# reasv/panoptikon

Measured on AMD Instinct MI355X. Metric: knn_queries_per_sec, higher is better.
Workload: dtype i8

## Files before the change

panoptikon_amd/csrc/pvs_api.hip:

```cpp
#include "pvs_index.hpp"

static thread_local std::string g_last_error;

pvs_status pvs_fail(pvs_status code, const char *fmt, ...) {
    char buf[512];
    va_list ap;
    va_start(ap, fmt);
    vsnprintf(buf, sizeof buf, fmt, ap);
    va_end(ap);
    g_last_error = buf;
    return code;
}
PVS_EXPORT const char *pvs_last_error(void) { return g_last_error.c_str(); }

namespace {
std::atomic<int64_t> g_dbg[PVS_DBG_COUNT];
const char *const g_dbg_names[PVS_DBG_COUNT] = {
    "sample_div",      "sample_j_div", "no_light_finalize", "force_light_finalize", "dense_per_query",     "no_direct_score",
    "no_page_rank",    "rrf_serial",   "rrf_full",          "rrf_trace",            "scan_no_wide128",     "scratch_idle_cap_mb",
    "scratch_bypass",  "rrf_digest",   "no_sparse",         "sparse_max",           "no_fused_agg",        "no_side_finalize",
    "rrf_host_rounds", "multi_host_pages", "prelude_stream", "dense_nq4", "marker_events", "no_direct_topk", "direct_max_mb", "direct_queries",
    "direct_unit", "direct_static_pct", "direct_max_nq", "dense_full_sort", "dense_page_first", "no_flag_poll", "poll_late_pages",
    "no_exact_wide", "no_agg8", "no_dense2", "comm_timeout_s", "comm_fail_local",
    "no_float_certify", "float_certify_queries", "float_certify_rows", "float_certify_trace", "float_certify_no_fold",
// ... 285 lines not shown
    }
    c.spans.clear();
    c.span_pool.clear();
    hipFree(c.d_qin);
    hipFree(c.d_qmat);
    hipFree(c.d_qpad);
    hipFree(c.d_direct);
    hipFree(c.d_qstage);
    hipFree(c.d_mask);
    hipFree(c.d_aux_masked);
    hipFree(c.d_qexact);
    hipFree(c.d_qinfo);
    hipFree(c.d_thr);
    hipFree(c.d_gmin);
    hipFree(c.d_cand_cnt);
    hipFree(c.d_seg);
    hipFree(c.d_seg_cnt);
    hipFree(c.d_cand);
    hipFree(c.d_flat_cnt);
    hipFree(c.d_fin_ub);
    hipFree(c.d_fin_surv);
    hipFree(c.d_fin_sort);
    c.d_fin_ub = c.d_fin_surv = nullptr;
    c.d_fin_sort = nullptr;
    hipFree(c.d_need_dense);
    if (c.h_need_dense) hipHostFree(c.h_need_dense);
    hipFree(c.d_out_ids);
    hipFree(c.d_out_dist);
    hipFree(c.d_out_count);
    pvs_dense_release(c.dense);
    pvs_group_work_release(c.gwork);
    if (c.done) hipEventDestroy(c.done);
    if (c.scanned) hipEventDestroy(c.scanned);
    if (c.preluded) hipEventDestroy(c.preluded);
    hipFree(c.d_loc_rec);
    hipFree(c.d_all_rec);
    if (c.h_all_flags) hipHostFree(c.h_all_flags);
    if (c.own_stream) hipStreamDestroy(c.own_stream);
    if (c.h_io) hipHostFree(c.h_io);
    if (c.h_cert) hipHostFree(c.h_cert);
    c = SearchCtx();
}

pvs_status ctx_pinned_io(SearchCtx &c, size_t bytes) {
    if (bytes <= c.h_io_cap) return PVS_OK;
    if (c.h_io) hipHostFree(c.h_io);
    c.h_io = nullptr;
    c.h_io_cap = 0;
    const size_t cap = pvs_round_up(std::max<size_t>(bytes, 1 << 16), 1 << 16);
    HIP_TRY(hipHostMalloc((void **)&c.h_io, cap, hipHostMallocDefault));
    c.h_io_cap = cap;
    return PVS_OK;
}

pvs_status ctx_fin_buffers(SearchCtx &c) {
    if (c.d_fin_ub && c.d_fin_surv && c.d_fin_sort) return PVS_OK;
    if (!c.d_fin_ub) HIP_TRY(pvs_malloc_retry((void **)&c.d_fin_ub, 4 * (size_t)PVS_SCAN_MAX_BATCH * PVS_CAND_CAP));
    if (!c.d_fin_surv) HIP_TRY(pvs_malloc_retry((void **)&c.d_fin_surv, 4 * (size_t)PVS_SCAN_MAX_BATCH * PVS_SURV_CAP));
    if (!c.d_fin_sort) HIP_TRY(pvs_malloc_retry((void **)&c.d_fin_sort, 8 * (size_t)PVS_SCAN_MAX_BATCH * PVS_SURV_CAP));
    return PVS_OK;
}

pvs_status ctx_prepare(pvs_index *ix, SearchCtx &c, uint32_t batch, uint32_t k, bool host_outputs) {
    if (ix->multi_stream) {
        if (!c.own_stream) HIP_TRY(hipStreamCreateWithFlags(&c.own_stream, hipStreamNonBlocking));
        c.stream = c.own_stream;
    } else {
        c.stream = ix->search_stream;
    }
    c.cur_mask = nullptr;
    if (!c.done) HIP_TRY(hipEventCreateWithFlags(&c.done, hipEventDisableTiming));
    if (!c.scanned) HIP_TRY(hipEventCreateWithFlags(&c.scanned, hipEventDisableTiming));
    if (!c.preluded) HIP_TRY(hipEventCreateWithFlags(&c.preluded, hipEventDisableTiming));
    c.side_finalize = false;
    if (!c.d_qmat) {
        HIP_TRY(pvs_malloc_retry((void **)&c.d_qin, (size_t)PVS_SCAN_MAX_BATCH * ix->dim * 4));
        HIP_TRY(pvs_malloc_retry((void **)&c.d_qmat, (size_t)PVS_SCAN_MAX_BATCH * ix->stride));
        HIP_TRY(pvs_malloc_retry((void **)&c.d_qpad, pvs_dense_exact_scratch_bytes(ix->stride, ix->esz)));
        HIP_TRY(pvs_malloc_retry((void **)&c.d_qexact, (size_t)PVS_SCAN_MAX_BATCH * ix->dim * 4));
        HIP_TRY(pvs_malloc_retry((void **)&c.d_qinfo, sizeof(QInfo) * PVS_SCAN_MAX_BATCH));
        HIP_TRY(pvs_malloc_retry((void **)&c.d_thr, 4 * PVS_SCAN_MAX_BATCH));
        HIP_TRY(pvs_malloc_retry((void **)&c.d_gmin, (size_t)4 * PVS_SCAN_MAX_BATCH * GMAX));
        HIP_TRY(pvs_malloc_retry((void **)&c.d_cand_cnt, 64));
        HIP_TRY(pvs_malloc_retry((void **)&c.d_seg, sizeof(uint2) * (size_t)PVS_SEG_PAIRS * PVS_SEG_CAP));
        HIP_TRY(pvs_malloc_retry((void **)&c.d_seg_cnt, 4 * (size_t)PVS_SEG_PAIRS * (PVS_SEG_CAP / PVS_WIDE_SEG_CAP)));
        HIP_TRY(pvs_malloc_retry((void **)&c.d_cand, sizeof(uint2) * (size_t)PVS_SCAN_MAX_BATCH * PVS_CAND_CAP));
        HIP_TRY(pvs_malloc_retry((void **)&c.d_flat_cnt, 4 * (size_t)PVS_SCAN_MAX_BATCH));
    }
    if (batch > c.flags_cap) {
        hipFree(c.d_need_dense);
        if (c.h_need_dense) hipHostFree(c.h_need_dense);
        c.d_need_dense = nullptr;
        c.h_need_dense = nullptr;
        uint32_t cap = (uint32_t)pvs_round_up(batch, 256);
        HIP_TRY(pvs_malloc_retry((void **)&c.d_need_dense, 8 * (size_t)cap));
        HIP_TRY(hipHostMalloc((void **)&c.h_need_dense, 8 * (size_t)cap, hipHostMallocDefault));
        c.flags_cap = cap;
    }
    if (host_outputs) {
        uint64_t need = (uint64_t)batch * k;
        if (need > c.out_cap || batch > c.out_batch_cap) {
            hipFree(c.d_out_ids);
            hipFree(c.d_out_dist);
            hipFree(c.d_out_count);
// ... 592 lines not shown
```

panoptikon_amd/csrc/pvs_index.hpp:

```cpp
#pragma once
#include <sched.h>

#include <algorithm>
#include <cmath>
#include <chrono>
#include <condition_variable>
#include <thread>

#include "pvs_kernels.hpp"

struct PendingChunk {
    uint32_t qoff, nb;
};

struct PageSplit {
    uint32_t at;
    int64_t *ids;
    float *dist;
    uint32_t *count, *h_flags, *h_seen;
};

struct TimedSpan {
    hipEvent_t a, b;
    int kind;
    uint64_t rows;
};

struct SearchCtx {
    std::vector<TimedSpan> spans;
    std::vector<TimedSpan> span_pool;
    hipStream_t stream = nullptr;
    hipStream_t own_stream = nullptr;
    hipEvent_t done = nullptr;
    hipEvent_t preluded = nullptr;
    hipEvent_t scanned = nullptr;
    bool side_finalize = false;
    bool busy = false;
    bool draining = false, finished = false;
    pvs_status fin_status = PVS_OK;
    std::string fin_err;
    uint8_t *d_qin = nullptr;
    uint8_t *d_qmat = nullptr;
    float *d_qpad = nullptr;
    void *d_direct = nullptr;
    const uint8_t *cur_mask = nullptr;
    uint8_t *d_mask = nullptr;
    float *d_aux_masked = nullptr;
    uint64_t mask_cap = 0;
    void *d_qstage = nullptr;
    size_t qstage_cap = 0;
    uint8_t *d_qexact = nullptr;
    QInfo *d_qinfo = nullptr;
    float *d_thr = nullptr;
    float *d_gmin = nullptr;
    uint32_t *d_cand_cnt = nullptr;
    uint2 *d_seg = nullptr;
    uint32_t *d_seg_cnt = nullptr;
    uint2 *d_cand = nullptr;
    uint32_t *d_flat_cnt = nullptr;
    uint32_t *d_fin_ub = nullptr, *d_fin_surv = nullptr;
    unsigned long long *d_fin_sort = nullptr;
    uint32_t *d_need_dense = nullptr;
    uint32_t *h_need_dense = nullptr;
    uint32_t flags_cap = 0;
    int64_t *d_out_ids = nullptr;
    float *d_out_dist = nullptr;
    uint32_t *d_out_count = nullptr;
    uint64_t out_cap = 0;
    uint32_t out_batch_cap = 0;
// ... 362 lines not shown
```

panoptikon_amd/csrc/pvs_kernels.hpp:

```cpp
#pragma once
#include <cstring>
#include "pvs_common.hpp"

hipError_t pvs_launch_norm2(int dtype, const uint8_t *rows, uint32_t stride, uint32_t dim, uint64_t row0, uint64_t n,
                            float *norm2, float *rnorm, hipStream_t s);
hipError_t pvs_launch_fill_f32(float *p, uint64_t n, float v, hipStream_t s);
hipError_t pvs_launch_scan_aux(const float *norm2, const float *rnorm, uint64_t row0, uint64_t n, float *scan_cos, float *scan_l2,
                               hipStream_t s);
hipError_t pvs_launch_rows_ingest(int mode, const void *src, uint32_t dim, uint32_t esz, uint64_t row0, uint64_t n, float scale,
                                  uint8_t *rows, uint32_t stride, hipStream_t s);
hipError_t pvs_launch_rows_gather(const uint8_t *rows, uint32_t stride, uint32_t row_bytes, uint64_t row0, uint64_t n, uint8_t *dst,
                                  hipStream_t s);
hipError_t pvs_launch_pick_rows(const void *src, uint32_t row_bytes, const uint32_t *idx, uint64_t m, void *dst, hipStream_t s);
hipError_t pvs_launch_rows_to_queries(int dtype, const uint8_t *rows, uint32_t stride, uint32_t dim, const uint32_t *idx, uint32_t m, void *out, hipStream_t s);
hipError_t pvs_launch_take_rows(const void *in, uint32_t elem_bytes, const uint32_t *global_row, uint64_t n_local, void *out, hipStream_t s);
hipError_t pvs_launch_quantize_flat(const float *src, uint64_t n, float scale, int8_t *dst, hipStream_t s);
hipError_t pvs_launch_absmax(const float *src, uint64_t n, float *d_out_bits, hipStream_t s);
hipError_t pvs_launch_synth(uint64_t seed, uint64_t row0, uint64_t n, uint32_t dim, float *out, hipStream_t s);
hipError_t pvs_launch_synth_clustered(uint64_t seed, uint64_t row0, uint64_t n, uint32_t dim, float *out, hipStream_t s);
hipError_t pvs_launch_iota_ids(int64_t *ids, uint64_t n, int64_t base, hipStream_t s);

hipError_t pvs_launch_prep_queries(int index_dtype, int qdtype, const void *queries, uint32_t batch,
                                   uint32_t batch_pad, uint32_t dim, uint32_t stride, float scale,
                                   int metric, uint8_t *qmat, void *qexact, QInfo *qinfo, uint32_t *need_dense, hipStream_t s);
// ... 97 lines not shown

hipError_t pvs_launch_void_thresholds(float *thr, const uint32_t *need_dense, uint32_t n, hipStream_t s);

hipError_t pvs_launch_kth(const float *vals, uint32_t per_query, uint32_t batch, uint32_t k, float *out,
                          hipStream_t s, const QInfo *qinfo = nullptr, int metric = 0);

struct FinalizeArgs {
    int dtype, metric;
    const uint8_t *rows;
    const float *norm2;
    const int64_t *ids;
    uint32_t stride, dim;
    uint64_t n_rows;
    const void *qexact;
    const QInfo *qinfo;
    const uint2 *seg;
    const uint32_t *seg_cnt;
    uint32_t n_segments, seg_queries;
    uint32_t seg_cap = PVS_SEG_CAP;
    uint2 *cand;
    uint32_t cand_cap;
    uint32_t batch, k;
    int64_t *out_ids;
    float *out_dist;
    uint32_t *out_count;
    uint32_t *need_dense;
    uint32_t *cand_seen = nullptr;
    const uint32_t *flat_cnt = nullptr;
    const float *thr = nullptr;
    const float *thr_all = nullptr;
    int null_ok = 0;
    uint32_t *h_flags = nullptr, *h_seen = nullptr;
    uint32_t split = UINT32_MAX;
    int64_t *out_ids2 = nullptr;
    float *out_dist2 = nullptr;
    uint32_t *out_count2 = nullptr, *h_flags2 = nullptr, *h_seen2 = nullptr;
    const uint32_t *trank = nullptr, *tinv = nullptr;
    uint32_t *w_ub = nullptr;
    uint32_t *w_surv = nullptr;
    unsigned long long *w_sort = nullptr;
    hipEvent_t ev_start = nullptr, ev_stop = nullptr;
};
hipError_t pvs_launch_finalize(const FinalizeArgs &a, hipStream_t s);

struct DenseWork {
    float *d_dist = nullptr;
    uint32_t *d_keys_in = nullptr, *d_keys_out = nullptr, *d_vals_in = nullptr, *d_vals_out = nullptr;
    void *d_temp = nullptr;
    size_t temp_bytes = 0;
    uint64_t cap_rows = 0, sort_rows = 0;
    uint32_t *d_sample = nullptr, *d_sample_out = nullptr, *d_ctl = nullptr, *h_ctl = nullptr;
    unsigned long long *d_comp = nullptr, *d_comp_out = nullptr;
    void *d_temp_page = nullptr;
    size_t temp_page_bytes = 0;
    uint32_t comp_cap = 0;
};
pvs_status pvs_dense_reserve(DenseWork &w, uint64_t n);
void pvs_dense_release(DenseWork &w);
struct DenseBounds {
    int have_gt = 0, have_lt = 0;
    double gt = 0.0, lt = 0.0;
};
pvs_status pvs_dense_topk(DenseWork &w, uint64_t n, uint32_t k, const int64_t *ids, int64_t *out_ids,
                          float *out_dist, uint32_t *out_count, hipStream_t s, const uint8_t *mask = nullptr,
                          DenseBounds bounds = DenseBounds(), const uint32_t *tinv = nullptr);
pvs_status pvs_build_tie_ranks(const int64_t *d_keys, uint64_t n, uint32_t *d_trank, uint32_t *d_tinv, hipStream_t s);
// ... 111 lines not shown
```

panoptikon_amd/csrc/pvs_kernels_scan.hip:

```cpp
#include <cstdlib>

#include <hip/hip_ext.h>
#include "pvs_kernels.hpp"
#include "pvs_rerank.hpp"
#include "pvs_scan_dispatch.hpp"

bool pvs_scan_supported(int dtype, uint32_t kslabs) {
    if (dtype == PVS_I8) return (kslabs >= 1 && kslabs <= 6) || kslabs == 8 || kslabs == 12;
    if (dtype == PVS_F16)
        return kslabs == 1 || kslabs == 2 || kslabs == 3 || kslabs == 4 || kslabs == 6 || kslabs == 8 || kslabs == 9 || kslabs == 10 || kslabs == 12;
    if (dtype == PVS_F32)
        return kslabs == 1 || kslabs == 2 || kslabs == 3 || kslabs == 4 || kslabs == 6 || kslabs == 8 || kslabs == 12 || kslabs == 16 || kslabs == 18 ||
               kslabs == 20 || kslabs == 24;
    return false;
}
bool pvs_scan_is_wide(int dtype, uint32_t qgroups, uint32_t kslabs) {
    const bool no128 = pvs_dbg(PVS_DBG_SCAN_NO_WIDE128) != 0;
    if (dtype != PVS_I8 || (qgroups == 4 && no128)) return false;
    return pvs_scan_wide_serves(qgroups, kslabs, 1);
}
uint32_t pvs_scan_wg_rows(int dtype, uint32_t qgroups, uint32_t kslabs) {
    if (pvs_scan_is_wide(dtype, qgroups, kslabs)) return pvs_scan_wide_rows(kslabs);
    return qgroups >= 4 ? 32u : 32u * (4u / qgroups);
}
// ... 235 lines not shown
    }
}

hipError_t pvs_launch_kth(const float *vals, uint32_t per_query, uint32_t batch, uint32_t k, float *out, hipStream_t s, const QInfo *qinfo, int metric) {
    const uint32_t bp = (batch + 31) / 32 * 32;
    hipLaunchKernelGGL(k_kth, dim3(bp), dim3(256), 0, s, vals, per_query, batch, k, out, qinfo, metric);
    return hipGetLastError();
}

struct FinK {
    const uint8_t *rows;
    const float *norm2;
    const int64_t *ids;
    const void *qexact;
    const QInfo *qinfo;
    const uint2 *seg;
    const uint32_t *seg_cnt;
    uint2 *cand;
    int64_t *out_ids;
    float *out_dist;
    uint32_t *out_count, *need_dense, *cand_seen;
    uint64_t n_rows;
    uint32_t stride, dim, cand_cap, k, n_segments, seg_queries, seg_cap;
    int metric;
    uint32_t *w_ub, *w_surv;
    unsigned long long *w_sort;
    const uint32_t *flat_cnt;
    const float *thr;
    const float *thr_all;
    int null_ok;
    uint32_t *h_flags, *h_seen;
    const uint32_t *trank, *tinv;
    uint32_t split;
    int64_t *out_ids2;
    float *out_dist2;
    uint32_t *out_count2, *h_flags2, *h_seen2;
};

constexpr int FIN_QMAX = 8192;
constexpr int FIN_LDS = PVS_CAND_CAP * 4 + PVS_SURV_CAP * 4 + 64 + FIN_QMAX;

__device__ static inline float cand_err(const FinK &a, const QInfo &qi, float aa) {
    return a.metric == PVS_COSINE ? qi.eA : qi.eA + qi.eR * aa;
}
template <int DT>
__device__ static inline float cand_key(const FinK &a, const QInfo &qi, uint32_t payload, float aa) {
    if constexpr (DT == PVS_I8) {
        const float d = (float)(int)payload;
        return a.metric == PVS_COSINE ? -d * __frcp_rn(__fsqrt_rn(aa)) : aa + (qi.bb - 2.0f * d);
    } else {
        return __builtin_bit_cast(float, payload);
    }
}

constexpr uint32_t FIN_SMALL_SORT = 512;
template <int DT, bool LIGHT>
__global__ __launch_bounds__(256) void k_finalize(FinK a) {
    extern __shared__ __attribute__((aligned(16))) uint8_t smem[];
    __shared__ uint32_t hist[256];
    __shared__ uint32_t s_misc_light[LIGHT ? 16 : 1];
    __shared__ unsigned long long s_sort_light[LIGHT ? FIN_SMALL_SORT : 1];
    const uint32_t q = blockIdx.x;
    uint32_t *const s_ub = LIGHT ? a.w_ub + (size_t)q * a.cand_cap : (uint32_t *)smem;
    uint32_t *const s_surv = LIGHT ? a.w_surv + (size_t)q * PVS_SURV_CAP : (uint32_t *)(smem + PVS_CAND_CAP * 4);
    uint32_t *const s_misc = LIGHT ? s_misc_light : (uint32_t *)(smem + PVS_CAND_CAP * 4) + PVS_SURV_CAP;
    unsigned long long *s_sort = LIGHT ? s_sort_light : (unsigned long long *)smem;

    const int tid = threadIdx.x;
#ifdef PVS_FIN_PROF
    unsigned long long fp[8] = {0, 0, 0, 0, 0, 0, 0, 0};
#define FIN_STAMP(i) fp[i] = __builtin_amdgcn_s_memrealtime()
#else
#define FIN_STAMP(i) do { } while (0)
#endif
    FIN_STAMP(0);
    const bool second = q >= a.split;
    const uint32_t qo = second ? q - a.split : q;
    uint32_t *const out_count = second ? a.out_count2 : a.out_count;
    uint32_t *const h_flags = second ? a.h_flags2 : a.h_flags;
    uint32_t *const h_seen = second ? a.h_seen2 : a.h_seen;
    int64_t *oid = (second ? a.out_ids2 : a.out_ids) + (size_t)qo * a.k;
    float *od = (second ? a.out_dist2 : a.out_dist) + (size_t)qo * a.k;
    if (a.null_ok && !a.flat_cnt && pvs_query_all_null(a.metric, a.qinfo[q].bb)) {
        if (tid == 0) {
            a.need_dense[q] = 3;
            if (h_flags) h_flags[qo] = 3;
            out_count[qo] = 0;
            if (a.cand_seen) a.cand_seen[q] = 0;
            if (h_seen) h_seen[qo] = 0;
        }
        return;
    }
    uint2 *const flat = a.cand + (size_t)q * a.cand_cap;
    constexpr uint32_t FIN_STAGE = 4096;
    static_assert(FIN_STAGE * 8 * 2 <= PVS_CAND_CAP * 4 && FIN_STAGE * 2 <= PVS_SURV_CAP, "staging areas overlap");
// ... 270 lines not shown
            oid[i] = -1;
            od[i] = __builtin_nanf("");
        }
    }
    if (tid == 0) {
        out_count[qo] = nout;
        a.need_dense[q] = tail ? 3 : 0;
        if (h_flags) h_flags[qo] = tail ? 3 : 0;
    }
}

hipError_t pvs_launch_finalize(const FinalizeArgs &f, hipStream_t s) {
    FinK k;
    k.rows = f.rows;
    k.norm2 = f.norm2;
    k.ids = f.ids;
    k.qexact = f.qexact;
    k.qinfo = f.qinfo;
    k.seg = f.seg;
    k.seg_cnt = f.seg_cnt;
    k.n_segments = f.n_segments;
    k.w_ub = f.w_ub;
    k.w_surv = f.w_surv;
    k.w_sort = f.w_sort;
    k.seg_queries = f.seg_queries;
    k.seg_cap = f.seg_cap;
    k.flat_cnt = f.flat_cnt;
    k.thr = f.thr;
    k.thr_all = f.thr_all;
    k.null_ok = f.null_ok;
    k.h_flags = f.h_flags;
    k.h_seen = f.h_seen;
    k.split = f.split;
    k.out_ids2 = f.out_ids2;
    k.out_dist2 = f.out_dist2;
    k.out_count2 = f.out_count2;
    k.h_flags2 = f.h_flags2;
    k.h_seen2 = f.h_seen2;
    k.trank = f.trank;
    k.tinv = f.tinv;
    k.cand = f.cand;
    k.out_ids = f.out_ids;
    k.out_dist = f.out_dist;
    k.out_count = f.out_count;
    k.need_dense = f.need_dense;
    k.cand_seen = f.cand_seen;
    k.n_rows = f.n_rows;
    k.stride = f.stride;
    k.dim = f.dim;
    k.cand_cap = f.cand_cap;
    k.k = f.k;
    k.metric = f.metric;
    static std::atomic<bool> configured{false};
    if (!configured.load(std::memory_order_acquire)) {
        hipError_t e = hipFuncSetAttribute((const void *)k_finalize<PVS_I8, false>, hipFuncAttributeMaxDynamicSharedMemorySize, FIN_LDS);
        if (e == hipSuccess)
            e = hipFuncSetAttribute((const void *)k_finalize<PVS_F16, false>, hipFuncAttributeMaxDynamicSharedMemorySize, FIN_LDS);
        if (e == hipSuccess)
            e = hipFuncSetAttribute((const void *)k_finalize<PVS_F32, false>, hipFuncAttributeMaxDynamicSharedMemorySize, FIN_LDS);
        if (e != hipSuccess) return e;
        configured.store(true, std::memory_order_release);
    }
    if ((((uint64_t)f.dim * (f.dtype == PVS_I8 ? 1u : 4u)) + 63u & ~63ull) > (uint64_t)FIN_QMAX) return hipErrorInvalidValue;
    const bool light = f.w_ub && f.w_surv && f.w_sort;
    const size_t qlds = ((size_t)f.dim * 4 + 63) & ~(size_t)63;
#define PVS_FIN_LAUNCH(kernel, lds)                                                                                  \
    do {                                                                                                             \
        if (f.ev_start || f.ev_stop)                                                                                 \
            hipExtLaunchKernelGGL(kernel, dim3(f.batch), dim3(256), lds, s, f.ev_start, f.ev_stop, 0, k);            \
        else                                                                                                         \
            hipLaunchKernelGGL(kernel, dim3(f.batch), dim3(256), lds, s, k);                                         \
    } while (0)
    if (light && f.dtype == PVS_I8)
        PVS_FIN_LAUNCH((k_finalize<PVS_I8, true>), 0);
    else if (light && f.dtype == PVS_F16)
        PVS_FIN_LAUNCH((k_finalize<PVS_F16, true>), qlds);
    else if (light)
        PVS_FIN_LAUNCH((k_finalize<PVS_F32, true>), qlds);
    else if (f.dtype == PVS_I8)
        PVS_FIN_LAUNCH((k_finalize<PVS_I8, false>), FIN_LDS);
    else if (f.dtype == PVS_F16)
        PVS_FIN_LAUNCH((k_finalize<PVS_F16, false>), FIN_LDS);
    else
        PVS_FIN_LAUNCH((k_finalize<PVS_F32, false>), FIN_LDS);
#undef PVS_FIN_LAUNCH
    return hipGetLastError();
}

__device__ static inline bool page_less(float da, int64_t ka, int64_t ia, float db, int64_t kb, int64_t ib) {
    const uint32_t sa = f32_sort_key(da), sb = f32_sort_key(db);
    if (sa != sb) return sa < sb;
    if (ka != kb) return ka > kb;
    return ia < ib;
}
struct MergePages {
    const uint8_t *ids, *dist, *cnt;
    const uint8_t *flags, *keys;
    size_t stride_ids, stride_dist, stride_cnt, stride_flags, stride_keys;
    __device__ const int64_t *ids_of(uint32_t w) const { return (const int64_t *)(ids + (size_t)w * stride_ids); }
    __device__ const float *dist_of(uint32_t w) const { return (const float *)(dist + (size_t)w * stride_dist); }
    __device__ const uint32_t *cnt_of(uint32_t w) const { return (const uint32_t *)(cnt + (size_t)w * stride_cnt); }
    __device__ const uint32_t *flags_of(uint32_t w) const { return (const uint32_t *)(flags + (size_t)w * stride_flags); }
    __device__ const int64_t *keys_of(uint32_t w) const { return (const int64_t *)(keys + (size_t)w * stride_keys); }
};
// ... 98 lines not shown
```

panoptikon_amd/csrc/pvs_search.hip:

```cpp
#include <chrono>
#include <cstring>
#include <new>
#include <string>

#include "pvs_index.hpp"

pvs_status validate_search(pvs_index *ix, const void *queries, pvs_dtype qdtype, uint32_t batch, uint32_t k,
                                  pvs_metric metric) {
    if (!ix) return pvs_fail(PVS_ERR_INVALID_ARG, "null index");
    if (ix->poisoned) return pvs_fail(PVS_ERR_STATE, PVS_POISONED_MSG);
    if (batch && !queries) return pvs_fail(PVS_ERR_INVALID_ARG, "null queries");
    if (k < 1) return pvs_fail(PVS_ERR_INVALID_ARG, "k must be a positive integer");
    if (k > (1u << 20)) return pvs_fail(PVS_ERR_INVALID_ARG, "k too large");
    if (metric != PVS_COSINE && metric != PVS_L2) return pvs_fail(PVS_ERR_INVALID_ARG, "unknown metric");
    if (qdtype == PVS_I8) {
        if (ix->dtype != PVS_I8) return pvs_fail(PVS_ERR_DIM_MISMATCH, "int8 query against a float index (element type mismatch)");
    } else if (qdtype == PVS_F32) {
        if (ix->dtype == PVS_I8 && !ix->scale_set)
            return pvs_fail(PVS_ERR_STATE, "f32 query on an int8 index needs the scale artifact");
    } else {
        return pvs_fail(PVS_ERR_INVALID_ARG, "queries must be f32 or int8");
    }
    return PVS_OK;
}
// ... 22 lines not shown
    const size_t qesz = qdtype == PVS_I8 ? 1 : 4;
    const uint8_t *qsrc = (const uint8_t *)d_queries + (size_t)qoff * ix->dim * qesz;
    HIP_TRY(pvs_launch_prep_queries((int)ix->dtype, qdtype, qsrc, nb, batch_pad, ix->dim, ix->stride, ix->scale, metric, c.d_qmat,
                                    c.d_qexact, c.d_qinfo, c.d_need_dense + qoff, on ? on : c.stream));
    return PVS_OK;
}

static pvs_status enqueue_fast_chunk(pvs_index *ix, SearchCtx &c, uint32_t qoff, uint32_t nb, uint32_t batch_pad, uint32_t k, int metric,
                                     int64_t *oid, float *od, uint32_t *oc, bool flat_rerun, bool side = false, hipStream_t prelude = nullptr,
                                     const PageSplit *split = nullptr) {
    if ((ix->multi_stream || side || pvs_dbg(PVS_DBG_FORCE_LIGHT_FINALIZE)) && !pvs_dbg(PVS_DBG_NO_LIGHT_FINALIZE)) PVS_TRY(ctx_fin_buffers(c));
    ScanArgs a;
    a.dtype = (int)ix->dtype;
    a.metric = metric;
    a.kslabs = ix->stride / PVS_KSLAB_BYTES;
    a.qgroups = batch_pad / 32;
    a.rows = ix->d_rows;
    a.aux = metric == PVS_COSINE ? ix->d_scan_cos : ix->d_scan_l2;
    if (c.cur_mask) {
        HIP_TRY(pvs_launch_mask_aux(a.aux, c.cur_mask, ix->n, ix->cap, c.d_aux_masked, c.stream));
        a.aux = c.d_aux_masked;
    }
    a.stride = ix->stride;
    a.n_rows = ix->n;
    a.qmat = c.d_qmat;
    a.qinfo = c.d_qinfo;
    a.thr = c.d_thr;
    a.seg = c.d_seg;
    a.seg_cnt = c.d_seg_cnt;
    a.gmin = c.d_gmin;
    const uint32_t wg_rows = pvs_scan_wg_rows(a.dtype, a.qgroups, a.kslabs);
    const uint32_t n_wgtiles = (uint32_t)((ix->n + wg_rows - 1) / wg_rows);
    double frac = nb <= 4 ? 1.0 / 32.0 : 1.0 / 16.0;
    if (pvs_dbg(PVS_DBG_SAMPLE_DIV) > 0) frac = 1.0 / (double)pvs_dbg(PVS_DBG_SAMPLE_DIV);
    const uint32_t j_div = pvs_dbg(PVS_DBG_SAMPLE_J_DIV) > 0 ? (uint32_t)pvs_dbg(PVS_DBG_SAMPLE_J_DIV) : 4u;
    uint32_t k_sel = k;
    if (ix->n >= (1ull << 18) && !flat_rerun) k_sel = std::min(k, std::max<uint32_t>(8, k / j_div));
    frac *= (double)k_sel / (double)k;
    frac = std::min(0.5, std::max(frac, 2.5 * (double)k_sel / (double)PVS_CAND_CAP));
    const uint64_t target_rows = std::min<uint64_t>(ix->n, std::max<uint64_t>((uint64_t)((double)ix->n * frac), 32768));
    const uint32_t want_tiles = (uint32_t)std::max<uint64_t>(1, (target_rows + wg_rows - 1) / wg_rows);
    a.tile_step = std::max<uint32_t>(1, n_wgtiles / want_tiles);
    const uint32_t n_samp = (n_wgtiles + a.tile_step - 1) / a.tile_step;
    if (k_sel < k) {
        const double share = std::min(1.0, (double)n_samp * wg_rows / (double)ix->n);
        const double expect = std::min(8.0 * k, (double)PVS_CAND_CAP / 2.5);
        k_sel = std::min<uint32_t>(k, std::max<uint32_t>(k_sel, (uint32_t)std::ceil(expect * share)));
    }
    const uint32_t per_cu_a = pvs_scan_wg_per_cu(a.dtype, a.qgroups, a.kslabs);
    const uint32_t spp = pvs_scan_segs_per_stream(a.dtype, a.qgroups, a.kslabs);
    a.grid = std::min<uint32_t>({n_samp, (uint32_t)ix->n_cu * per_cu_a, GMAX / (spp * pvs_scan_gmin_max(a.dtype, a.qgroups, a.kslabs))});
    a.mode = 0;
    a.gmin_per_lane = pvs_scan_gmin_max(a.dtype, a.qgroups, a.kslabs);
    while (a.gmin_per_lane > 1 && (uint64_t)a.grid * spp * (a.gmin_per_lane / 2) >= std::max<uint64_t>(16ull * k_sel, 1024)) a.gmin_per_lane /= 2;
    a.groups_per_query = a.grid * spp * a.gmin_per_lane;
    hipStream_t ps = prelude ? prelude : c.stream;
    const bool bound_ev = pvs_dbg(PVS_DBG_MARKER_EVENTS) == 0;
    if (bound_ev) {
        (void)span_bound(ix, c, 0, (uint64_t)n_samp * wg_rows, &a.ev_start, &a.ev_stop);
        HIP_TRY(pvs_launch_scan(a, ps));
        a.ev_start = a.ev_stop = nullptr;
    } else {
        span_begin(ix, c, 0, (uint64_t)n_samp * wg_rows, ps);
        HIP_TRY(pvs_launch_scan(a, ps));
        span_end(ix, c, ps);
    }
    HIP_TRY(pvs_launch_kth(c.d_gmin, a.groups_per_query, nb, k_sel, c.d_thr, ps, c.d_qinfo, metric));
    if (prelude) {
// ... 54 lines not shown
    f.out_ids = oid;
    f.out_dist = od;
    f.out_count = oc;
    f.need_dense = c.d_need_dense + qoff;
    f.cand_seen = c.d_need_dense + c.flags_cap + qoff;
    if (flat_rerun) f.flat_cnt = c.d_flat_cnt;
    f.h_flags = c.h_need_dense + qoff;
    f.h_seen = c.h_need_dense + c.flags_cap + qoff;
    if (split) {
        f.split = split->at;
        f.out_ids2 = split->ids;
        f.out_dist2 = split->dist;
        f.out_count2 = split->count;
        f.h_flags2 = split->h_flags;
        f.h_seen2 = split->h_seen;
    }
    if (k_sel < k) f.thr = c.d_thr;
    f.thr_all = c.d_thr;
    f.null_ok = ix->null_built_n.load(std::memory_order_acquire) == ix->n && ix->null_weird[metric == PVS_L2 ? 1 : 0] == 0;
    if (order_tinv(ix)) {
        f.trank = ix->d_trank;
        f.tinv = ix->d_tinv;
    }
    hipStream_t fs = c.stream;
    if (side && f.w_ub) {
        if (!scanned) {
            HIP_TRY(hipEventRecord(c.scanned, c.stream));
            scanned = c.scanned;
        }
        HIP_TRY(hipStreamWaitEvent(ix->fin_stream, scanned, 0));
        fs = ix->fin_stream;
        c.side_finalize = true;
    }
    if (bound_ev) {
        (void)span_bound(ix, c, 2, 0, &f.ev_start, &f.ev_stop);
        HIP_TRY(pvs_launch_finalize(f, fs));
    } else {
        span_begin(ix, c, 2, 0, fs);
        HIP_TRY(pvs_launch_finalize(f, fs));
        span_end(ix, c, fs);
    }
    return PVS_OK;
}

bool pvs_direct_route(const pvs_index *ix, uint32_t k, uint32_t batch) {
    if (ix->forced_path != 0 || ix->n == 0 || pvs_dbg(PVS_DBG_NO_DIRECT_TOPK)) return false;
    if (batch > 1 && pvs_dbg(PVS_DBG_DIRECT_MAX_NQ) > 0 && (int64_t)batch > pvs_dbg(PVS_DBG_DIRECT_MAX_NQ)) return false;
    if (!pvs_direct_supported((int)ix->dtype, ix->stride, ix->esz, k, batch)) return false;
    const uint64_t lim_mb = pvs_dbg(PVS_DBG_DIRECT_MAX_MB) > 0 ? (uint64_t)pvs_dbg(PVS_DBG_DIRECT_MAX_MB) : PVS_DIRECT_CROSSOVER_MB;
    return ix->n * (uint64_t)ix->stride <= (lim_mb << 20);
}
bool direct_ok(const pvs_index *ix, const SearchCtx &c, uint32_t batch, uint32_t k) { return batch >= 1 && batch <= PVS_DIRECT_MAX_NQ && pvs_direct_route(ix, k, batch); }
pvs_status enqueue_direct(pvs_index *ix, SearchCtx &c, const void *d_queries, int qdtype, uint32_t batch, uint32_t k, int metric, int64_t *oid, float *od,
                          uint32_t *oc, uint8_t *h_page) {
    if (!c.d_direct) {
        const uint64_t bytes = pvs_direct_work_bytes((uint32_t)ix->n_cu);
        HIP_TRY(pvs_malloc_retry(&c.d_direct, bytes));
        HIP_TRY(hipMemsetAsync(c.d_direct, 0, bytes, c.stream));
    }
    PVS_TRY(prep_chunk(ix, c, d_queries, qdtype, 0, batch, 32, metric));
    DirectArgs d;
    d.dtype = (int)ix->dtype;
    d.metric = metric;
    d.rows = ix->d_rows;
    d.norm2 = ix->d_norm2;
    d.ids = ix->d_ids;
    d.stride = ix->stride;
    d.dim = ix->dim;
    d.n_rows = ix->n;
    d.qexact = c.d_qexact;
    d.qinfo = c.d_qinfo;
    if (order_tinv(ix)) {
        d.trank = ix->d_trank;
// ... 10 lines not shown
    d.h_flags = c.h_need_dense;
    d.h_seen = c.h_need_dense + c.flags_cap;
    d.null_ok = ix->null_built_n.load(std::memory_order_acquire) == ix->n && ix->null_weird[metric == PVS_L2 ? 1 : 0] == 0;
    d.n_cu = (uint32_t)ix->n_cu;
    if (h_page) {
        const size_t bk = (size_t)batch * k;
        d.h_out_ids = (int64_t *)h_page;
        d.h_out_dist = (float *)(h_page + bk * 8);
        d.h_out_count = (uint32_t *)(h_page + bk * 12);
        d.h_out_rows = (uint32_t *)(h_page + bk * 12 + 64);
    }
    (void)span_bound(ix, c, 1, ix->n, &d.ev_start, &d.ev_stop);
    HIP_TRY(pvs_launch_direct_topk(d, c.stream));
    ix->direct_queries += batch;
    pvs_dbg_add(PVS_DBG_DIRECT_QUERIES, batch);
    return PVS_OK;
}

pvs_status prep_slot(pvs_index *ix, SearchCtx &c, const void *d_queries, int qdtype, uint32_t slot, uint32_t nb, uint32_t batch_pad, int metric) {
    if (slot + batch_pad > PVS_SCAN_MAX_BATCH || slot + nb > c.flags_cap) return pvs_fail(PVS_ERR_INVALID_ARG, "query slots [%u, +%u) outside the context", slot, batch_pad);
    const size_t qesz = ix->dtype == PVS_I8 ? 1 : 4;
    HIP_TRY(pvs_launch_prep_queries((int)ix->dtype, qdtype, d_queries, nb, batch_pad, ix->dim, ix->stride, ix->scale, metric,
                                    c.d_qmat + (size_t)slot * ix->stride, c.d_qexact + (size_t)slot * ix->dim * qesz, c.d_qinfo + slot,
                                    c.d_need_dense + slot, c.stream));
    return PVS_OK;
}

pvs_status enqueue_joined_pass(pvs_index *ix, SearchCtx &c, uint32_t nb, uint32_t k, int metric, int64_t *oid, float *od, uint32_t *oc,
                               const PageSplit *split) {
    const uint32_t batch_pad = nb <= 32 ? 32 : nb <= 64 ? 64 : nb <= 128 ? 128 : 256;
    const bool side = !ix->multi_stream && c.stream == ix->search_stream && !pvs_dbg(PVS_DBG_NO_SIDE_FINALIZE);
    c.side_finalize = false;
    PVS_TRY(enqueue_fast_chunk(ix, c, 0, nb, batch_pad, k, metric, oid, od, oc, false, side, nullptr, split));
    HIP_TRY(hipEventRecord(c.done, c.side_finalize ? ix->fin_stream : c.stream));
    return PVS_OK;
}

pvs_status search_enqueue(pvs_index *ix, SearchCtx &c, const void *d_queries, int qdtype, uint32_t batch, uint32_t k,
                                 int metric, int64_t *d_out_ids, float *d_out_dist, uint32_t *d_out_count, bool *used_fast, bool side_finalize) {
    const bool fast = fast_path_ok(ix, k);
    *used_fast = fast;
    if (!fast && ix->forced_path == 2) return pvs_fail(PVS_ERR_UNSUPPORTED, "filter-scan path not available for this index / k");
    if (ix->n == 0) {
        HIP_TRY(hipMemsetAsync(c.d_need_dense, 0, 4 * (size_t)batch, c.stream));
        HIP_TRY(hipMemsetAsync(d_out_count, 0, 4 * (size_t)batch, c.stream));
        HIP_TRY(hipMemsetAsync(d_out_ids, 0xff, 8 * (size_t)batch * k, c.stream));
        HIP_TRY(pvs_launch_fill_f32(d_out_dist, (uint64_t)batch * k, __builtin_nanf(""), c.stream));
        HIP_TRY(hipEventRecord(c.done, c.stream));
        return PVS_OK;
    }
    if (fast) PVS_TRY(pvs_ensure_null_rows(ix));
    if (direct_ok(ix, c, batch, k)) {
        if (!fast) PVS_TRY(pvs_ensure_null_rows(ix));
        *used_fast = true;
        PVS_TRY(enqueue_direct(ix, c, d_queries, qdtype, batch, k, metric, d_out_ids, d_out_dist, d_out_count));
        HIP_TRY(hipEventRecord(c.done, c.stream));
        return PVS_OK;
    }
    const uint32_t pass_max = fast ? pvs_scan_max_batch((int)ix->dtype, ix->stride / PVS_KSLAB_BYTES) : PVS_MAX_BATCH;
    for (uint32_t qoff = 0; qoff < batch; qoff += pass_max) {
        const uint32_t nb = std::min(pass_max, batch - qoff);
        const uint32_t batch_pad = nb <= 32 ? 32 : nb <= 64 ? 64 : nb <= 128 ? 128 : 256;
        const bool side = fast && side_finalize && batch <= pass_max && !ix->multi_stream && c.stream == ix->search_stream &&
                          !pvs_dbg(PVS_DBG_NO_SIDE_FINALIZE);
        hipStream_t prelude = side && !c.cur_mask && pvs_dbg(PVS_DBG_PRELUDE_STREAM) ? ix->pre_stream : nullptr;
        PVS_TRY(prep_chunk(ix, c, d_queries, qdtype, qoff, nb, batch_pad, metric, prelude));
        int64_t *oid = d_out_ids + (size_t)qoff * k;
// ... 2 lines not shown
        if (!fast) {
            const bool per_query = pvs_dbg(PVS_DBG_DENSE_PER_QUERY) != 0;
            if (nb >= 2 && pvs_select_supported(k) && !per_query) {
                const uint32_t per = (uint32_t)std::max<uint64_t>(1, std::min<uint64_t>((uint64_t)nb, (1ull << 31) / (4 * std::max<uint64_t>(ix->n, 1))));
                float *d_m = nullptr;
                HIP_TRY(pvs_scratch_alloc((void **)&d_m, (size_t)ix->n * per * 4));
                pvs_status st = PVS_OK;
                for (uint32_t off = 0; off < nb && st == PVS_OK; off += per) {
                    const uint32_t nbb = std::min(per, nb - off);
                    const uint32_t pad = nbb <= 32 ? 32 : nbb <= 64 ? 64 : 128;
                    st = prep_chunk(ix, c, d_queries, qdtype, qoff + off, nbb, pad, metric);
                    if (st == PVS_OK) st = dense_chunk(ix, c, nbb, pad, metric, d_m);
                    if (st == PVS_OK)
                        st = pvs_select_topk(d_m, ix->n, nbb, nbb, k, c.cur_mask, ix->d_ids, nullptr, oid + (size_t)off * k, od + (size_t)off * k, oc + off, c.stream, order_tinv(ix));
                }
                pvs_scratch_free_on(d_m, c.stream);
                PVS_TRY(st);
                ix->dense_queries += nb;
                continue;
            }
            for (uint32_t q = 0; q < nb; q++) PVS_TRY(dense_one(ix, c, q, k, metric, oid + (size_t)q * k, od + (size_t)q * k, oc + q));
            continue;
        }
        PVS_TRY(enqueue_fast_chunk(ix, c, qoff, nb, batch_pad, k, metric, oid, od, oc, false, side, prelude));
    }
    HIP_TRY(hipEventRecord(c.done, c.side_finalize ? ix->fin_stream : c.stream));
    return PVS_OK;
}

pvs_status search_fallbacks(pvs_index *ix, SearchCtx &c, const void *d_queries, int qdtype, uint32_t batch, uint32_t k,
                                   int metric, int64_t *d_out_ids, float *d_out_dist, uint32_t *d_out_count) {
    uint32_t n_dense = 0, n_rerun = 0;
    uint64_t seen = 0;
    for (uint32_t q = 0; q < batch; q++) {
        n_rerun += c.h_need_dense[q] == 2 ? 1 : 0;
        seen += c.h_need_dense[c.flags_cap + q];
    }
    if (n_rerun && fast_path_ok(ix, k)) {
        const uint32_t pass_max = pvs_scan_max_batch((int)ix->dtype, ix->stride / PVS_KSLAB_BYTES);
        for (uint32_t qoff = 0; qoff < batch; qoff += pass_max) {
            const uint32_t nb = std::min(pass_max, batch - qoff);
            bool any = false;
            for (uint32_t q = 0; q < nb; q++) any |= c.h_need_dense[qoff + q] == 2;
            if (!any) continue;
            const uint32_t batch_pad = nb <= 32 ? 32 : nb <= 64 ? 64 : nb <= 128 ? 128 : 256;
            PVS_TRY(prep_chunk(ix, c, d_queries, qdtype, qoff, nb, batch_pad, metric));
            HIP_TRY(hipMemcpyAsync(c.d_need_dense + qoff, c.h_need_dense + qoff, 4 * (size_t)nb, hipMemcpyHostToDevice, c.stream));
            PVS_TRY(enqueue_fast_chunk(ix, c, qoff, nb, batch_pad, k, metric, d_out_ids + (size_t)qoff * k, d_out_dist + (size_t)qoff * k,
                                       d_out_count + qoff, true));
        }
        HIP_TRY(hipMemcpyAsync(c.h_need_dense, c.d_need_dense, 4 * (size_t)batch, hipMemcpyDeviceToHost, c.stream));
        HIP_TRY(hipStreamSynchronize(c.stream));
        ix->flat_reruns += n_rerun;
    }
    uint32_t n_tail = 0;
    for (uint32_t q = 0; q < batch; q++) n_tail += c.h_need_dense[q] == 3 ? 1 : 0;
    if (n_tail) {
        const uint32_t pass_max = pvs_scan_max_batch((int)ix->dtype, ix->stride / PVS_KSLAB_BYTES);
        for (uint32_t qoff = 0; qoff < batch; qoff += pass_max) {
            const uint32_t nb = std::min(pass_max, batch - qoff);
            bool any = false;
            for (uint32_t q = 0; q < nb; q++) any |= c.h_need_dense[qoff + q] == 3;
            if (!any) continue;
            const uint32_t batch_pad = nb <= 32 ? 32 : nb <= 64 ? 64 : nb <= 128 ? 128 : 256;
            PVS_TRY(prep_chunk(ix, c, d_queries, qdtype, qoff, nb, batch_pad, metric));
            HIP_TRY(hipMemcpyAsync(c.d_need_dense + qoff, c.h_need_dense + qoff, 4 * (size_t)nb, hipMemcpyHostToDevice, c.stream));
            PVS_TRY(pvs_launch_null_tails(ix, c, metric, c.d_need_dense + qoff, c.h_need_dense + qoff, nb, k, d_out_ids + (size_t)qoff * k, d_out_dist + (size_t)qoff * k,
                                          d_out_count + qoff));
        }
// ... 86 lines not shown
```

panoptikon_amd/csrc/pvs_search_device.hip:

```cpp
#include <chrono>
#include <cstring>
#include <new>
#include <string>

#include "pvs_index.hpp"

static bool join_applies(pvs_index *ix, uint32_t batch, uint32_t k) {
    if (pvs_dbg(PVS_DBG_JOIN_US) <= 0 || ix->multi_stream || ix->dtype != PVS_I8 || ix->n == 0) return false;
    const uint32_t pass_max = pvs_scan_max_batch((int)ix->dtype, ix->stride / PVS_KSLAB_BYTES);
    return batch > PVS_DIRECT_MAX_NQ && 2 * batch <= pass_max && pass_max == PVS_SCAN_MAX_BATCH && fast_path_ok(ix, k);
}
static uint32_t pass_pad(uint32_t nb) { return nb <= 32 ? 32 : nb <= 64 ? 64 : nb <= 128 ? 128 : 256; }

struct JoinPartner {
    uint32_t ticket, nb;
    int64_t *ids;
    float *dist;
    uint32_t *count;
};
static pvs_status join_launch_locked(pvs_index *ix, const JoinPartner *p) {
    auto &j = ix->join;
    if (!j.held) return PVS_OK;
    j.held = false;
    SearchCtx &c = ix->ctx[j.ticket];
    SearchCtx *m = p ? &ix->ctx[p->ticket] : nullptr;
    const uint32_t nb = j.nb + (p ? p->nb : 0);
    auto body = [&]() -> pvs_status {
        HIP_TRY(hipSetDevice(ix->device));
        PageSplit sp{};
        if (m) sp = PageSplit{j.nb, p->ids, p->dist, p->count, m->h_need_dense, m->h_need_dense + m->flags_cap};
        PVS_TRY(enqueue_joined_pass(ix, c, nb, j.k, j.metric, j.ids, j.dist, j.count, m ? &sp : nullptr));
        if (m) HIP_TRY(hipEventRecord(m->done, c.side_finalize ? ix->fin_stream : c.stream));
        return PVS_OK;
    };
    const pvs_status st = body();
    if (st == PVS_OK) {
        pvs_dbg_add(m ? PVS_DBG_JOINED_PASSES : PVS_DBG_JOIN_ALONE_PASSES, 1);
        if (m) pvs_dbg_add(PVS_DBG_JOINED_QUERIES, nb);
        return PVS_OK;
    }
    const std::string why = pvs_last_error();
    (void)hipStreamSynchronize(c.stream);
    (void)hipStreamSynchronize(ix->fin_stream);
    c.j_status = st;
    c.j_err = why;
    if (m) {
        m->j_status = st;
        m->j_err = why;
    }
    return st;
}
pvs_status pvs_join_flush_(pvs_index *ix) {
    if (!ix || is_multi(ix)) return PVS_OK;
    std::lock_guard<std::mutex> lk(ix->join.mu);
    return join_launch_locked(ix, nullptr);
}
static void join_window(pvs_index *ix) {
    auto &j = ix->join;
    (void)hipSetDevice(ix->device);
    std::unique_lock<std::mutex> lk(j.mu);
    while (!j.stop) {
        if (!j.held) {
            j.cv.wait(lk);
            continue;
        }
// ... 512 lines not shown
```

Before: 127,000.

## Split joined-pass finalize so first partner completes early on main stream

When two queries' batches are joined into one pass, finalize now launches in two parts. The first partner's queries run on the search stream and signal their own done event early. The second partner's queries run from an offset q0, on the side finalize stream when side finalize is active. A tail event defers later waits on the side stream until a follow-up pass or fallback actually needs them. The wide (256-pad) pass also uses a larger sampling fraction and a different j_div for threshold estimation. The aim is lower latency for the first joined request, at the cost of extra launches and more complex cross-stream ordering.

```diff
diff --git a/panoptikon_amd/csrc/pvs_api.hip b/panoptikon_amd/csrc/pvs_api.hip
--- a/panoptikon_amd/csrc/pvs_api.hip
+++ b/panoptikon_amd/csrc/pvs_api.hip
@@ -341,6 +341,7 @@
     pvs_group_work_release(c.gwork);
     if (c.done) hipEventDestroy(c.done);
     if (c.scanned) hipEventDestroy(c.scanned);
+    if (c.tail) hipEventDestroy(c.tail);
     if (c.preluded) hipEventDestroy(c.preluded);
     hipFree(c.d_loc_rec);
     hipFree(c.d_all_rec);
@@ -378,7 +379,12 @@
         c.stream = ix->search_stream;
     }
     c.cur_mask = nullptr;
+    if (c.tail_pending) {
+        HIP_TRY(hipStreamWaitEvent(c.stream, c.tail, 0));
+        c.tail_pending = false;
+    }
     if (!c.done) HIP_TRY(hipEventCreateWithFlags(&c.done, hipEventDisableTiming));
+    if (!c.tail) HIP_TRY(hipEventCreateWithFlags(&c.tail, hipEventDisableTiming));
     if (!c.scanned) HIP_TRY(hipEventCreateWithFlags(&c.scanned, hipEventDisableTiming));
     if (!c.preluded) HIP_TRY(hipEventCreateWithFlags(&c.preluded, hipEventDisableTiming));
     c.side_finalize = false;
diff --git a/panoptikon_amd/csrc/pvs_index.hpp b/panoptikon_amd/csrc/pvs_index.hpp
--- a/panoptikon_amd/csrc/pvs_index.hpp
+++ b/panoptikon_amd/csrc/pvs_index.hpp
@@ -18,6 +18,7 @@
     int64_t *ids;
     float *dist;
     uint32_t *count, *h_flags, *h_seen;
+    hipEvent_t first_done;
 };
 
 struct TimedSpan {
@@ -35,6 +36,8 @@
     hipEvent_t preluded = nullptr;
     hipEvent_t scanned = nullptr;
     bool side_finalize = false;
+    hipEvent_t tail = nullptr;
+    bool tail_pending = false;
     bool busy = false;
     bool draining = false, finished = false;
     pvs_status fin_status = PVS_OK;
diff --git a/panoptikon_amd/csrc/pvs_kernels.hpp b/panoptikon_amd/csrc/pvs_kernels.hpp
--- a/panoptikon_amd/csrc/pvs_kernels.hpp
+++ b/panoptikon_amd/csrc/pvs_kernels.hpp
@@ -153,6 +153,7 @@
     int null_ok = 0;
     uint32_t *h_flags = nullptr, *h_seen = nullptr;
     uint32_t split = UINT32_MAX;
+    uint32_t q0 = 0;
     int64_t *out_ids2 = nullptr;
     float *out_dist2 = nullptr;
     uint32_t *out_count2 = nullptr, *h_flags2 = nullptr, *h_seen2 = nullptr;
diff --git a/panoptikon_amd/csrc/pvs_kernels_scan.hip b/panoptikon_amd/csrc/pvs_kernels_scan.hip
--- a/panoptikon_amd/csrc/pvs_kernels_scan.hip
+++ b/panoptikon_amd/csrc/pvs_kernels_scan.hip
@@ -291,6 +291,7 @@
     uint32_t *h_flags, *h_seen;
     const uint32_t *trank, *tinv;
     uint32_t split;
+    uint32_t q0;
     int64_t *out_ids2;
     float *out_dist2;
     uint32_t *out_count2, *h_flags2, *h_seen2;
@@ -319,7 +320,7 @@
     __shared__ uint32_t hist[256];
     __shared__ uint32_t s_misc_light[LIGHT ? 16 : 1];
     __shared__ unsigned long long s_sort_light[LIGHT ? FIN_SMALL_SORT : 1];
-    const uint32_t q = blockIdx.x;
+    const uint32_t q = a.q0 + blockIdx.x;
     uint32_t *const s_ub = LIGHT ? a.w_ub + (size_t)q * a.cand_cap : (uint32_t *)smem;
     uint32_t *const s_surv = LIGHT ? a.w_surv + (size_t)q * PVS_SURV_CAP : (uint32_t *)(smem + PVS_CAND_CAP * 4);
     uint32_t *const s_misc = LIGHT ? s_misc_light : (uint32_t *)(smem + PVS_CAND_CAP * 4) + PVS_SURV_CAP;
@@ -656,6 +657,7 @@
     k.h_flags = f.h_flags;
     k.h_seen = f.h_seen;
     k.split = f.split;
+    k.q0 = f.q0;
     k.out_ids2 = f.out_ids2;
     k.out_dist2 = f.out_dist2;
     k.out_count2 = f.out_count2;
@@ -686,14 +688,16 @@
         configured.store(true, std::memory_order_release);
     }
     if ((((uint64_t)f.dim * (f.dtype == PVS_I8 ? 1u : 4u)) + 63u & ~63ull) > (uint64_t)FIN_QMAX) return hipErrorInvalidValue;
+    if (f.q0 >= f.batch) return hipErrorInvalidValue;
+    const uint32_t nwg = f.batch - f.q0;
     const bool light = f.w_ub && f.w_surv && f.w_sort;
     const size_t qlds = ((size_t)f.dim * 4 + 63) & ~(size_t)63;
 #define PVS_FIN_LAUNCH(kernel, lds)                                                                                  \
     do {                                                                                                             \
         if (f.ev_start || f.ev_stop)                                                                                 \
-            hipExtLaunchKernelGGL(kernel, dim3(f.batch), dim3(256), lds, s, f.ev_start, f.ev_stop, 0, k);            \
+            hipExtLaunchKernelGGL(kernel, dim3(nwg), dim3(256), lds, s, f.ev_start, f.ev_stop, 0, k);                \
         else                                                                                                         \
-            hipLaunchKernelGGL(kernel, dim3(f.batch), dim3(256), lds, s, k);                                         \
+            hipLaunchKernelGGL(kernel, dim3(nwg), dim3(256), lds, s, k);                                             \
     } while (0)
     if (light && f.dtype == PVS_I8)
         PVS_FIN_LAUNCH((k_finalize<PVS_I8, true>), 0);
diff --git a/panoptikon_amd/csrc/pvs_search.hip b/panoptikon_amd/csrc/pvs_search.hip
--- a/panoptikon_amd/csrc/pvs_search.hip
+++ b/panoptikon_amd/csrc/pvs_search.hip
@@ -78,8 +78,10 @@
     const uint32_t wg_rows = pvs_scan_wg_rows(a.dtype, a.qgroups, a.kslabs);
     const uint32_t n_wgtiles = (uint32_t)((ix->n + wg_rows - 1) / wg_rows);
     double frac = nb <= 4 ? 1.0 / 32.0 : 1.0 / 16.0;
+    const bool wide_pass = batch_pad == 256;
+    if (wide_pass) frac = 1.0 / 8.0;
     if (pvs_dbg(PVS_DBG_SAMPLE_DIV) > 0) frac = 1.0 / (double)pvs_dbg(PVS_DBG_SAMPLE_DIV);
-    const uint32_t j_div = pvs_dbg(PVS_DBG_SAMPLE_J_DIV) > 0 ? (uint32_t)pvs_dbg(PVS_DBG_SAMPLE_J_DIV) : 4u;
+    const uint32_t j_div = pvs_dbg(PVS_DBG_SAMPLE_J_DIV) > 0 ? (uint32_t)pvs_dbg(PVS_DBG_SAMPLE_J_DIV) : wide_pass ? 8u : 4u;
     uint32_t k_sel = k;
     if (ix->n >= (1ull << 18) && !flat_rerun) k_sel = std::min(k, std::max<uint32_t>(8, k / j_div));
     frac *= (double)k_sel / (double)k;
@@ -200,13 +202,28 @@
         fs = ix->fin_stream;
         c.side_finalize = true;
     }
+    FinalizeArgs f1 = f;
+    hipStream_t fs1 = fs;
+    if (split && split->first_done) {
+        f1.batch = split->at;
+        if (!ix->multi_stream && !force_light) {
+            f1.w_ub = f1.w_surv = nullptr;
+            f1.w_sort = nullptr;
+        }
+        fs1 = c.stream;
+        f.q0 = split->at;
+    }
     if (bound_ev) {
-        (void)span_bound(ix, c, 2, 0, &f.ev_start, &f.ev_stop);
+        (void)span_bound(ix, c, 2, 0, &f1.ev_start, &f1.ev_stop);
+        HIP_TRY(pvs_launch_finalize(f1, fs1));
+    } else {
+        span_begin(ix, c, 2, 0, fs1);
+        HIP_TRY(pvs_launch_finalize(f1, fs1));
+        span_end(ix, c, fs1);
+    }
+    if (split && split->first_done) {
+        HIP_TRY(hipEventRecord(split->first_done, c.stream));
         HIP_TRY(pvs_launch_finalize(f, fs));
-    } else {
-        span_begin(ix, c, 2, 0, fs);
-        HIP_TRY(pvs_launch_finalize(f, fs));
-        span_end(ix, c, fs);
     }
     return PVS_OK;
 }
@@ -283,7 +300,7 @@
     const bool side = !ix->multi_stream && c.stream == ix->search_stream && !pvs_dbg(PVS_DBG_NO_SIDE_FINALIZE);
     c.side_finalize = false;
     PVS_TRY(enqueue_fast_chunk(ix, c, 0, nb, batch_pad, k, metric, oid, od, oc, false, side, nullptr, split));
-    HIP_TRY(hipEventRecord(c.done, c.side_finalize ? ix->fin_stream : c.stream));
+    if (!split) HIP_TRY(hipEventRecord(c.done, c.side_finalize ? ix->fin_stream : c.stream));
     return PVS_OK;
 }
 
@@ -352,9 +369,15 @@
                                    int metric, int64_t *d_out_ids, float *d_out_dist, uint32_t *d_out_count) {
     uint32_t n_dense = 0, n_rerun = 0;
     uint64_t seen = 0;
+    bool any_flag = false;
     for (uint32_t q = 0; q < batch; q++) {
         n_rerun += c.h_need_dense[q] == 2 ? 1 : 0;
         seen += c.h_need_dense[c.flags_cap + q];
+        any_flag |= c.h_need_dense[q] != 0;
+    }
+    if (any_flag && c.tail_pending) {
+        HIP_TRY(hipStreamWaitEvent(c.stream, c.tail, 0));
+        c.tail_pending = false;
     }
     if (n_rerun && fast_path_ok(ix, k)) {
         const uint32_t pass_max = pvs_scan_max_batch((int)ix->dtype, ix->stride / PVS_KSLAB_BYTES);
diff --git a/panoptikon_amd/csrc/pvs_search_device.hip b/panoptikon_amd/csrc/pvs_search_device.hip
--- a/panoptikon_amd/csrc/pvs_search_device.hip
+++ b/panoptikon_amd/csrc/pvs_search_device.hip
@@ -28,9 +28,15 @@
     auto body = [&]() -> pvs_status {
         HIP_TRY(hipSetDevice(ix->device));
         PageSplit sp{};
-        if (m) sp = PageSplit{j.nb, p->ids, p->dist, p->count, m->h_need_dense, m->h_need_dense + m->flags_cap};
+        if (m) sp = PageSplit{j.nb, p->ids, p->dist, p->count, m->h_need_dense, m->h_need_dense + m->flags_cap, c.done};
         PVS_TRY(enqueue_joined_pass(ix, c, nb, j.k, j.metric, j.ids, j.dist, j.count, m ? &sp : nullptr));
-        if (m) HIP_TRY(hipEventRecord(m->done, c.side_finalize ? ix->fin_stream : c.stream));
+        if (m) {
+            HIP_TRY(hipEventRecord(m->done, c.side_finalize ? ix->fin_stream : c.stream));
+            if (c.side_finalize) {
+                HIP_TRY(hipEventRecord(c.tail, ix->fin_stream));
+                c.tail_pending = true;
+            }
+        }
         return PVS_OK;
     };
     const pvs_status st = body();
```

New measurement: 131,700, median of 6. 1.04x the previous value.
